# giuspugl/COSMOMAP2

Measured on AMD Instinct MI355X. Metric: TOD samples/s through P^T N^-1 P, higher is better.
Workload: dtype f64

## Files before the change

cosmomap2_amd/build.py:

```python
import glob
import os
import subprocess
import sys
from concurrent.futures import ThreadPoolExecutor

HERE = os.path.dirname(os.path.abspath(__file__))
CSRC = os.path.join(HERE, "csrc")
OBJ = os.path.join(HERE, "csrc", "build")
LIB = os.path.join(HERE, "libcosmomap2_hip.so")
ARCH = "gfx950"
HIPCC = os.environ.get("HIPCC", "/opt/rocm/bin/hipcc")
FLAGS = ["--offload-arch=" + ARCH, "-O3", "-fPIC", "-std=c++17", "-ffp-contract=off",
         "-fno-fast-math", "-Wall", "-Wno-unused-result", "-munsafe-fp-atomics"]


FMA_OK = {"cm2_overlap_save.hip"}


STAMP = os.path.join(HERE, "libcosmomap2_hip.sources.sha16")


def source_hash():
    import hashlib
    h = hashlib.sha256()
    files = sorted(glob.glob(os.path.join(CSRC, "*.hip")) + glob.glob(os.path.join(CSRC, "*.h")) +
                   glob.glob(os.path.join(HERE, "..", "include", "*.h")), key=os.path.basename)
    for f in files:
        h.update(os.path.basename(f).encode() + b"\0")
        h.update(open(f, "rb").read())
    return h.hexdigest()[:16]


def library_stamp():
    at_build = open(STAMP).read().strip() if os.path.exists(STAMP) else None
    if os.environ.get("CM2_LIB_PATH"):
        at_build = "variant:" + os.path.basename(os.environ["CM2_LIB_PATH"])
    return {"sources_sha16_at_build": at_build, "sources_sha16_now": source_hash(),
            "library_matches_sources": at_build is not None and at_build == source_hash()}


def _newer(target, deps):
    if not os.path.exists(target):
        return True
    t = os.path.getmtime(target)
    return any(os.path.getmtime(d) > t for d in deps)


def compile_command(src, obj):
    flags = list(FLAGS) + os.environ.get("CM2_EXTRA_HIPCC_FLAGS", "").split()
    if os.path.basename(src) in FMA_OK:
        flags[flags.index("-ffp-contract=off")] = "-ffp-contract=fast"
    return [HIPCC] + flags + ["-Rpass-analysis=kernel-resource-usage", "-c", src, "-o", obj]


def build(force=False, verbose=True, allow_spills=None):
    from cosmomap2_amd import kernel_resources as KR
    os.makedirs(OBJ, exist_ok=True)
    srcs = sorted(glob.glob(os.path.join(CSRC, "*.hip")))
    hdrs = glob.glob(os.path.join(CSRC, "*.h")) + \
        glob.glob(os.path.join(HERE, "..", "include", "*.h"))
    jobs = []
    objs = []
    for s in srcs:
        o = os.path.join(OBJ, os.path.basename(s)[:-4] + ".o")
        objs.append(o)
        res = os.path.join(OBJ, os.path.basename(s)[:-4] + ".resources.json")
        if force or _newer(o, [s] + hdrs) or not os.path.exists(res):
            jobs.append((s, compile_command(s, o)))
    for f in os.listdir(OBJ):
        stem = f.split(".")[0]
        if (f.endswith(".o") or f.endswith(".resources.json")) and \
                not os.path.exists(os.path.join(CSRC, stem + ".hip")):
            os.remove(os.path.join(OBJ, f))

    def run(job):
        src, cmd = job
        if verbose:
            print(" ".join(cmd), flush=True)
        p = subprocess.run(cmd, stderr=subprocess.PIPE, text=True)
        rest = [ln for ln in p.stderr.splitlines() if "-Rpass-analysis=kernel-resource-usage" not in ln]
        if rest and (verbose or p.returncode):
            print("\n".join(rest), file=sys.stderr, flush=True)
        if p.returncode:
            raise subprocess.CalledProcessError(p.returncode, cmd)
        KR.store(os.path.basename(src), p.stderr)

    if jobs:
        with ThreadPoolExecutor(max_workers=min(4, len(jobs))) as ex:
            list(ex.map(run, jobs))
    if jobs or force or _newer(LIB, objs):
        cmd = [HIPCC, "--offload-arch=" + ARCH, "-shared", "-o", LIB] + objs + \
            ["-L/opt/rocm/lib", "-lrocfft", "-Wl,-rpath,/opt/rocm/lib"]
        if verbose:
            print(" ".join(cmd), flush=True)
        subprocess.check_call(cmd)
        with open(STAMP, "w") as fh:
            fh.write(source_hash() + "\n")
    elif not os.path.exists(STAMP):
        with open(STAMP, "w") as fh:
            fh.write(source_hash() + "\n")
    rows = KR.load_all()
    if jobs:
        prof = os.path.join(HERE, "..", "profiles")
        if os.path.isdir(prof):
            with open(os.path.join(prof, "kernel_resources.md"), "w") as fh:
                fh.write("# Register / scratch / LDS use of every kernel in libcosmomap2_hip.so\n\n"
                         "Written by `cosmomap2_amd/build.py` from hipcc's `-Rpass-analysis=kernel-resource-usage` "
                         "remarks of the compile that produced the shipped objects (gfx950). The build fails "
                         "when a kernel matching `kernel_resources.NO_SPILL` spills.\n\n")
                fh.write(KR.table(KR.own_kernels(rows)) + "\n")
    bad = KR.offenders(rows)
    if bad:
        msg = "default-path kernels spill registers: " + ", ".join(
            "%s (%d VGPRs, %d SGPRs spilled, %d B/lane scratch)" % (
                r["kernel"], r.get("vgpr_spill", 0), r.get("sgpr_spill", 0),
                r.get("scratch_bytes_per_lane", 0)) for r in bad)
        if allow_spills if allow_spills is not None else os.environ.get("CM2_ALLOW_SPILLS"):
            print("WARNING: " + msg, file=sys.stderr)
        else:
            raise RuntimeError(msg)
    return LIB


if __name__ == "__main__":
    build(force="--force" in sys.argv)
    print(LIB)
```

cosmomap2_amd/csrc/cm2_overlap_save.hip:

```cpp
#include "cm2_overlap_save.h"

#include <hipcub/hipcub.hpp>
#include <cstring>
#include <memory>
#include <mutex>

using namespace cm2;

namespace {

constexpr double kCos32[32] = {1.0, 0.9807852804032304, 0.9238795325112867, 0.8314696123025452, 0.7071067811865476, 0.5555702330196022, 0.3826834323650898, 0.19509032201612828, 0.0, -0.19509032201612828, -0.3826834323650898, -0.5555702330196022, -0.7071067811865476, -0.8314696123025452, -0.9238795325112867, -0.9807852804032304, -1.0, -0.9807852804032304, -0.9238795325112867, -0.8314696123025452, -0.7071067811865476, -0.5555702330196022, -0.3826834323650898, -0.19509032201612828, 0.0, 0.19509032201612828, 0.3826834323650898, 0.5555702330196022, 0.7071067811865476, 0.8314696123025452, 0.9238795325112867, 0.9807852804032304};
constexpr double kSin32[32] = {0.0, 0.19509032201612828, 0.3826834323650898, 0.5555702330196022, 0.7071067811865476, 0.8314696123025452, 0.9238795325112867, 0.9807852804032304, 1.0, 0.9807852804032304, 0.9238795325112867, 0.8314696123025452, 0.7071067811865476, 0.5555702330196022, 0.3826834323650898, 0.19509032201612828, 0.0, -0.19509032201612828, -0.3826834323650898, -0.5555702330196022, -0.7071067811865476, -0.8314696123025452, -0.9238795325112867, -0.9807852804032304, -1.0, -0.9807852804032304, -0.9238795325112867, -0.8314696123025452, -0.7071067811865476, -0.5555702330196022, -0.3826834323650898, -0.19509032201612828};

__host__ __device__ constexpr int ilog2(int r) { return r <= 1 ? 0 : 1 + ilog2(r >> 1); }

template <int R>
__host__ __device__ constexpr int brev(int m)
{
    int out = 0;
    for (int b = 0; b < ilog2(R); ++b) out |= ((m >> b) & 1) << (ilog2(R) - 1 - b);
    return out;
}

template <class T> __device__ __forceinline__ T ld_list(const T *p) { return __builtin_nontemporal_load(p); }
// ... 302 lines not shown
            ca[i] = ab_own[o + i * kT];
            cb[i] = ab_prt[(PT - 1) * kT - o - i * kT];
        }
    };
    request(0);
    __builtin_amdgcn_sched_barrier(0);
#pragma unroll
    for (int j = 0; j < H; ++j) {
        wp[H + j] = zr[reg_slot<16>(H + j)];
        wp[j] = zi[reg_slot<16>(H + j)];
    }
    if (special) {
#pragma unroll
        for (int j = 0; j < H; ++j) {
            xbuf[t * H + j] = zr[reg_slot<16>(j)];
            xbuf[(8 + t) * H + j] = zi[reg_slot<16>(j)];
        }
    }
    __syncthreads();
    if (!special) {
        double *__restrict__ pp = buf + 33 * (263 - t) + 31;
#pragma unroll
        for (int m0 = 0; m0 < H; m0 += BP) {
            if (m0 > 0) request(m0);
#pragma unroll
            for (int i0 = 0; i0 < BP; i0 += 4) {
                double pre[4], pim[4];
#pragma unroll
                for (int i = 0; i < 4; ++i) {
                    pre[i] = pp[-(m0 + i0 + i)];
                    pim[i] = pp[-H - (m0 + i0 + i)];
                }
#pragma unroll
                for (int i = 0; i < 4; ++i) {
                    const int m = m0 + i0 + i, sl = reg_slot<16>(m);
                    const double a = ca[i0 + i].x, b = ca[i0 + i].y, ap = cb[i0 + i].x, bp = cb[i0 + i].y;
                    const double nr = a * zr[sl] + b * pim[i];
                    const double ni = a * zi[sl] + b * pre[i];
                    const double qr = ap * pre[i] + bp * zi[sl];
                    const double qi = ap * pim[i] + bp * zr[sl];
                    zr[sl] = nr;
                    zi[sl] = ni;
                    pp[-m] = qr;
                    pp[-H - m] = qi;
                }
            }
            __builtin_amdgcn_sched_barrier(0);
        }
    } else {
        const int tl = t == 0 ? 0 : 8 - t;
        const double *__restrict__ up = buf + 33 * (7 - t) + 47;
#pragma unroll
        for (int m0 = 0; m0 < H; m0 += BP) {
            if (m0 > 0) request(m0);
#pragma unroll
            for (int i = 0; i < BP; ++i) {
                const int m = m0 + i, sl = reg_slot<16>(m);
                const int ms = t == 0 ? (m == 0 ? 0 : H - m) : H - 1 - m;
                const double pre_ = xbuf[tl * H + ms], pim_ = xbuf[(8 + tl) * H + ms];
                const double nr = ca[i].x * zr[sl] + ca[i].y * pim_;
                const double ni = ca[i].x * zi[sl] + ca[i].y * pre_;
                zr[sl] = nr;
                zi[sl] = ni;
                const int mu = PT - 1 - m, su = reg_slot<16>(mu);
                const double ure = up[-mu], uim = up[-mu - H];
                zr[su] = cb[i].x * wp[mu] + cb[i].y * uim;
                zi[su] = cb[i].x * wp[mu - H] + cb[i].y * ure;
            }
            __builtin_amdgcn_sched_barrier(0);
        }
    }
    __syncthreads();
    if (!special) {
#pragma unroll
        for (int j = 0; j < H; ++j) {
            zr[reg_slot<16>(H + j)] = wp[H + j];
            zi[reg_slot<16>(H + j)] = wp[j];
        }
    }
    __syncthreads();
}


template <int PT, int MODE, bool BUF>
__global__ __launch_bounds__(kT, PT == 16 ? 4 : 2) void k_os_real(
    const WinDesc *__restrict__ wins, int nwin, const double2 *__restrict__ Wtw,
    const double2 *Wtw_inv, const double2 *__restrict__ AB, const uint32_t *__restrict__ lst_k,
    const uint16_t *__restrict__ lst_q, const ListHdr *__restrict__ hdrs,
    const uint32_t *__restrict__ tabs, int rmax, const double *__restrict__ v,
    double *__restrict__ out, uint32_t nbytes, const IListHdr *__restrict__ ihdrs,
    const uint32_t *__restrict__ iflags OS_STAMP_PARAM)
{
    using G = Geo<PT>;
    constexpr int N = G::N, H = PT / 2;
    __amdgpu_buffer_rsrc_t v_rs, o_rs;
    if constexpr (BUF) {
        v_rs = __builtin_amdgcn_make_buffer_rsrc(const_cast<double *>(v), 0, (int)nbytes, 0x00020000);
        o_rs = __builtin_amdgcn_make_buffer_rsrc(out, 0, (int)nbytes, 0x00020000);
    }
    auto gather = [&](uint32_t k) -> double {
        if constexpr (BUF) {
            const v2u_t r = __builtin_amdgcn_raw_buffer_load_b64(v_rs, k * 8u, 0, 0);
            return __builtin_bit_cast(double, r);
        } else {
            return ld_gather(v + (k != kInvalidSample ? k : 0u));
        }
    };
    auto keep = [&](uint32_t k, double x) -> double {
        if constexpr (BUF) return x;
        return k != kInvalidSample ? x : 0.0;
    };
    extern __shared__ double buf[];
    uint32_t *__restrict__ tab_lds = reinterpret_cast<uint32_t *>(buf + G::LDSD);
    const int t = threadIdx.x;
    const int per_xcd = (nwin + 7) / 8;
    const int win = (blockIdx.x & 7) * per_xcd + (blockIdx.x >> 3);
    if (win >= nwin) return;
    const WinDesc wd = wins[win];
    const int64_t w0 = wd.start - kHalo;
    const int wave = __builtin_amdgcn_readfirstlane(t >> 6);
    OS_STAMP(0);

    auto list_args = [&](int l) {
        ListArgs la;
        const int64_t e0 = (int64_t)win * G::PER + G::list_off(l);
        la.k = nullptr;
        la.q = nullptr;
        la.hdr = nullptr;
        la.tab = nullptr;
        if constexpr (MODE == 1) la.k = lst_k + e0;
        if constexpr (MODE == 1 || MODE == 2) la.q = lst_q + e0;
        if constexpr (MODE == 2) {
            la.hdr = hdrs + ((int64_t)win * G::NLIST + l);
            la.tab = tabs + ((int64_t)win * G::NLIST + l) * rmax;
        }
        return la;
    };

    double zr[PT], zi[PT];
    if constexpr (MODE == 0) {
#pragma unroll
        for (int h = 0; h < 2; ++h) {
            double vv[PT];
#pragma unroll
            for (int u = 0; u < PT; ++u) {
                const int64_t ts = w0 + (int64_t)h * N + t + u * kT;
                vv[u] = (ts >= wd.lo && ts < wd.hi) ? v[ts] : 0.0;
            }
#pragma unroll
            for (int u = 0; u < PT; ++u) buf[t + u * kT] = vv[u];
            __syncthreads();
            const double2 *__restrict__ sp = reinterpret_cast<const double2 *>(buf) + t;
#pragma unroll
            for (int m = 0; m < H; ++m) {
                const double2 p = sp[256 * m];
                zr[h * H + m] = p.x;
                zi[h * H + m] = p.y;
            }
            __syncthreads();
        }
    } else if constexpr (MODE == 3) {
        const IListHdr *__restrict__ h0 = ihdrs + (int64_t)win * 2;
        const uint32_t *__restrict__ pl = reinterpret_cast<const uint32_t *>(lst_q + (int64_t)win * G::PER);
        uint32_t fw[2], pp[PT];
        {
            tab_dma(tabs + ((int64_t)win * 2) * rmax, tab_lds, rmax, wave, t);
            fw[0] = iflags[((int64_t)win * 2) * 512 + t];
            fw[1] = iflags[((int64_t)win * 2) * 512 + 256 + t];
        }
        const uint32_t nv = h0->nvalid;
        const int wb0 = h0->wbase[wave], wb1 = h0->wbase[4 + wave];
#pragma unroll
        for (int m = 0; m < PT; ++m) pp[m] = pl[t + kT * m];
        __syncthreads();
        double va[PT], vb[PT];
        {
            uint32_t kk[PT];
            idecode<PT>(fw[0], tab_lds, wb0, nv, 0u, t, kk);
#pragma unroll
            for (int u = 0; u < PT; ++u) va[u] = keep(kk[u], gather(kk[u]));
        }
        __builtin_amdgcn_sched_barrier(0);
        {
            uint32_t kk[PT];
            idecode<PT>(fw[1], tab_lds, wb1, nv, (uint32_t)N, t, kk);
#pragma unroll
            for (int u = 0; u < PT; ++u) vb[u] = keep(kk[u], gather(kk[u]));
        }
        __builtin_amdgcn_sched_barrier(0);
#pragma unroll
        for (int j = 0; j < 2; ++j) {
#pragma unroll
            for (int u = 0; u < PT; ++u) buf[slot_of<PT>(t, u)] = j ? vb[u] : va[u];
            if (j == 1) {
                int tj = t;
                asm volatile("" : "+v"(tj));
#pragma unroll
                for (int m = 0; m < PT; ++m) pp[m] = pl[tj + kT * m];
            }
            __syncthreads();
#pragma unroll
            for (int m = 0; m < PT; ++m) {
                const uint32_t lo = (pp[m] & 0xFFFFu) - (uint32_t)(j * N), hi = (pp[m] >> 16) - (uint32_t)(j * N);
                const bool inl = lo < (uint32_t)N, inh = hi < (uint32_t)N;
                const double x = buf[inl ? lo : 0u], y = buf[inh ? hi : 0u];
                if (j == 0) {
                    zr[m] = inl ? x : 0.0;
                    zi[m] = inh ? y : 0.0;
                } else {
                    zr[m] = inl ? x : zr[m];
                    zi[m] = inh ? y : zi[m];
                }
            }
            __syncthreads();
        }
    } else {
        const ListArgs l0 = list_args(0), l1 = list_args(1);
        uint32_t qa[PT / 2], qb[PT / 2], ka[PT], kb[PT];
        uint32_t nva = 0, nvb = 0;
        int wba = -1, wbb = -1;
        if constexpr (MODE == 2) {
            nva = l0.hdr->nvalid;
            nvb = l1.hdr->nvalid;
            wba = l0.hdr->wbase[wave];
            wbb = l1.hdr->wbase[wave];
            tab_dma(l0.tab, tab_lds, rmax, wave, t);
            tab_dma(l1.tab, tab_lds + rmax, rmax, wave, t);
        }
        q_request<PT>(l0.q, t, qa);
        if constexpr (MODE == 1) {
#pragma unroll
            for (int u = 0; u < PT; ++u) ka[u] = ld_list(l0.k + slot_of<PT>(t, u));
        }
        q_request<PT>(l1.q, t, qb);
        if constexpr (MODE == 1) {
#pragma unroll
            for (int u = 0; u < PT; ++u) kb[u] = ld_list(l1.k + slot_of<PT>(t, u));
        }
        if constexpr (MODE == 2) {
            __syncthreads();
            OS_STAMP(6);
            rc_decode<PT>(qa, tab_lds, wba, nva, t, ka);
        }
        __builtin_amdgcn_sched_barrier(0);
        double va[PT], vv[PT];
        if constexpr (MODE == 2) rc_decode<PT>(qb, tab_lds + rmax, wbb, nvb, t, kb);
#pragma unroll
        for (int u = 0; u < PT; ++u) va[u] = gather(ka[u]);
#pragma unroll
        for (int u = 0; u < PT; ++u) vv[u] = gather(kb[u]);
        __builtin_amdgcn_sched_barrier(0);
#pragma unroll
        for (int u = 0; u < PT; ++u) buf[q_word(qa, u) & 0x7FFFu] = keep(ka[u], va[u]);
        OS_STAMP(7);
        __syncthreads();
        {
            const double2 *__restrict__ sp = reinterpret_cast<const double2 *>(buf) + t;
#pragma unroll
            for (int m = 0; m < H; ++m) {
                const double2 p = sp[256 * m];
                zr[m] = p.x;
                zi[m] = p.y;
            }
        }
        __syncthreads();
#pragma unroll
        for (int u = 0; u < PT; ++u) buf[q_word(qb, u) & 0x7FFFu] = keep(kb[u], vv[u]);
        __syncthreads();
        {
            const double2 *__restrict__ sp = reinterpret_cast<const double2 *>(buf) + t;
#pragma unroll
            for (int m = 0; m < H; ++m) {
                const double2 p = sp[256 * m];
                zr[H + m] = p.x;
                zi[H + m] = p.y;
            }
        }
        __syncthreads();
    }

    OS_STAMP(1);
    const double2 w_a = Wtw[t];
    const double2 w_b = Wtw[PT * (t & 15)];

    OS_XF(reg_fwd<PT, PT, 0>(zr, zi, w_a));
    OS_XF(reg_exchange<PT, 1, 2, PT>(zr, buf, t));
    OS_XF(reg_exchange<PT, 1, 2, PT>(zi, buf, t));
    OS_XF(reg_fwd<PT, 16, 0>(zr, zi, w_b));
    OS_XF(if constexpr (PT == 32) reg_fwd<PT, 16, 16>(zr, zi, w_b));
    OS_XF(reg_exchange<PT, 2, 3, 16>(zr, buf, t));
    OS_XF(reg_exchange<PT, 2, 3, 16>(zi, buf, t));
    const double2 *ab = AB + (int64_t)wd.blk * N + t;
    OS_XF(dft_sub<PT, 16, 0>(zr, zi));
    OS_XF(if constexpr (PT == 32) dft_sub<PT, 16, 16>(zr, zi));
    OS_STAMP(2);
    OS_XF(partner_filter_half<PT, (MODE == 1 && !BUF) ? 4 : 8>(zr, zi, buf, reinterpret_cast<double *>(tab_lds + 2 * rmax),
                                                               t, ab, AB + (int64_t)wd.blk * N));
    (void)ab;
    OS_STAMP(3);
    OS_XF(dit_sub<PT, 16, 0>(zi, zr));
    OS_XF(if constexpr (PT == 32) dit_sub<PT, 16, 16>(zi, zr));
    const double2 w_bi = Wtw_inv[PT * (t & 15)], w_ai = Wtw_inv[t];
    OS_XF(reg_exchange<PT, 3, 2, 0>(zr, buf, t));
    OS_XF(reg_exchange<PT, 3, 2, 0>(zi, buf, t));
    asm volatile("" : : "v"(w_bi.x), "v"(w_bi.y), "v"(w_ai.x), "v"(w_ai.y));
    __builtin_amdgcn_sched_barrier(0);
    if constexpr (MODE == 3) {
        constexpr int ER3 = G::RLEN / kT, NP = PT - 8;
        int l1 = 1;
        asm volatile("" : "+s"(l1));
        const IListHdr *h1 = ihdrs + (int64_t)win * 2 + l1;
        const uint32_t *tg = tabs + ((int64_t)win * 2 + l1) * rmax;
        const uint32_t *fg = iflags + ((int64_t)win * 2 + l1) * 512 + t;
        const uint32_t nv1 = h1->nvalid;
        uint32_t fr[G::RR], rp[NP];
        const uint32_t *rl = reinterpret_cast<const uint32_t *>(lst_q + (int64_t)win * G::PER + 2 * N);
        {
            tab_dma(tg, tab_lds + rmax, rmax, wave, t);
#pragma unroll
            for (int j = 0; j < G::RR; ++j) fr[j] = fg[256 * j];
            int t0 = t;
            asm volatile("" : "+v"(t0));
#pragma unroll
            for (int m = 0; m < NP; ++m) rp[m] = rl[t0 + kT * m];
        }
        __builtin_amdgcn_sched_barrier(0);
        OS_XF(reg_inv<PT, 16, 0>(zr, zi, w_bi));
        OS_XF(if constexpr (PT == 32) reg_inv<PT, 16, 16>(zr, zi, w_bi));
        OS_XF(reg_exchange<PT, 2, 1, 16>(zr, buf, t));
        OS_XF(reg_exchange<PT, 2, 1, 16>(zi, buf, t));
        OS_XF(reg_inv<PT, PT, 0>(zr, zi, w_ai));
        OS_STAMP(4);
#pragma unroll
        for (int j = 0; j < G::RR; ++j) {
            if (j > 0) {
                __syncthreads();
                int tj = t;
                asm volatile("" : "+v"(tj));
#pragma unroll
                for (int m = 0; m < NP; ++m) rp[m] = rl[tj + kT * m];
            }
#pragma unroll
            for (int m = 0; m < NP; ++m) {
                const uint32_t lo = (rp[m] & 0xFFFFu) - (uint32_t)(j * G::RLEN), hi = (rp[m] >> 16) - (uint32_t)(j * G::RLEN);
                buf[lo < (uint32_t)G::RLEN ? lo : (uint32_t)N] = zr[brev<PT>(m + 4)];
                buf[hi < (uint32_t)G::RLEN ? hi : (uint32_t)N + 1u] = zi[brev<PT>(m + 4)];
            }
            __syncthreads();
            uint32_t ks3[ER3];
            idecode<ER3>(fr[j], tab_lds + rmax, h1->wbase[4 * j + wave], nv1, (uint32_t)(j * G::RLEN), t, ks3);
            double rv[ER3];
#pragma unroll
            for (int u = 0; u < ER3; ++u) rv[u] = buf[slot_of<ER3>(t, u)];
#pragma unroll
            for (int u = 0; u < ER3; ++u) {
                if constexpr (BUF) {
                    __builtin_amdgcn_raw_buffer_store_b64(__builtin_bit_cast(v2u_t, rv[u]), o_rs, ks3[u] * 8u, 0, 0);
                } else {
                    if (ks3[u] != kInvalidSample) st_result(out + ks3[u], rv[u]);
                }
            }
        }
    } else {
    constexpr int ER = G::RLEN / kT;
    uint32_t qs[ER / 2], ks[ER];
    uint32_t nvs = 0;
    int wbs = -1;
    auto request_results = [&](int j, auto &qq, auto &kq, uint32_t &nv, int &wb, uint32_t *tdst) {
        if constexpr (MODE != 0) {
            int lj = 2 + j;
            asm volatile("" : "+s"(lj));
            const ListArgs ls = list_args(lj);
            if constexpr (MODE == 2) {
                nv = ls.hdr->nvalid;
                wb = ls.hdr->wbase[wave];
                tab_dma(ls.tab, tdst, rmax, wave, t);
            }
            q_request<ER>(ls.q, t, qq);
            (void)kq;
        }
    };
    constexpr bool EARLY = MODE == 2 || (MODE == 1 && BUF);
    uint32_t qs1[ER / 2];
    uint32_t nv1 = 0;
    int wb1 = -1;
    request_results(0, qs, ks, nvs, wbs, tab_lds);
    __builtin_amdgcn_sched_barrier(0);
    OS_XF(reg_inv<PT, 16, 0>(zr, zi, w_bi));
    OS_XF(if constexpr (PT == 32) reg_inv<PT, 16, 16>(zr, zi, w_bi));
    OS_XF(reg_exchange<PT, 2, 1, 16>(zr, buf, t));
    OS_XF(reg_exchange<PT, 2, 1, 16>(zi, buf, t));
    OS_XF(reg_inv<PT, PT, 0>(zr, zi, w_ai));
    OS_STAMP(4);
#pragma unroll
    for (int j = 0; j < G::RR; ++j) {
        const uint32_t *tabj = tab_lds + (EARLY && j > 0 ? rmax : 0);
        if (j > 0) {
            __syncthreads();
            if constexpr (EARLY) {
#pragma unroll
                for (int i = 0; i < ER / 2; ++i) qs[i] = qs1[i];
                nvs = nv1;
                wbs = wb1;
            } else {
                request_results(j, qs, ks, nvs, wbs, tab_lds);
                if constexpr (MODE == 2) __syncthreads();
            }
        }
        if constexpr (MODE == 2) rc_decode<ER>(qs, tabj, wbs, nvs, t, ks);
        double2 *__restrict__ sp = reinterpret_cast<double2 *>(buf) + t;
#pragma unroll
        for (int mm = 0; mm < G::RSLOTS; ++mm) {
            const int m = 4 + j * G::RSLOTS + mm;
            sp[256 * mm] = make_double2(zr[brev<PT>(m)], zi[brev<PT>(m)]);
        }
        if constexpr (MODE == 1) {
            const ListArgs ls = list_args(2 + j);
#pragma unroll
            for (int u = 0; u < ER; ++u) ks[u] = ld_list(ls.k + slot_of<ER>(t, u));
        }
        __syncthreads();
        if constexpr (EARLY)
            if (j + 1 < G::RR) request_results(j + 1, qs1, ks, nv1, wb1, tab_lds + rmax);
        if constexpr (MODE == 0) {
#pragma unroll
            for (int u = 0; u < ER; ++u) {
                const int e = t + u * kT;
                const int64_t o = (int64_t)j * G::RLEN + e;
                if (o < wd.len) out[wd.start + o] = buf[e];
            }
        } else {
            double rv[ER];
#pragma unroll
            for (int u = 0; u < ER; ++u) rv[u] = buf[q_word(qs, u) & 0x7FFFu];
#pragma unroll
            for (int u = 0; u < ER; ++u) {
                if constexpr (BUF) {
                    __builtin_amdgcn_raw_buffer_store_b64(__builtin_bit_cast(v2u_t, rv[u]), o_rs, ks[u] * 8u, 0, 0);
                } else {
                    if (ks[u] != kInvalidSample) st_result(out + ks[u], rv[u]);
                }
            }
        }
    }
    }
    OS_STAMP(5);
}

template <int PT>
__global__ __launch_bounds__(256) void k_real_keys(const WinDesc *__restrict__ wins, int64_t w0,
                                                    int64_t nw, const uint32_t *__restrict__ idx,
                                                    uint32_t *__restrict__ keys,
                                                    uint16_t *__restrict__ vals)
{
    using G = Geo<PT>;
    const int64_t total = nw * G::PER;
    const int64_t stride = (int64_t)gridDim.x * blockDim.x;
    for (int64_t g = (int64_t)blockIdx.x * blockDim.x + threadIdx.x; g < total; g += stride) {
        const int64_t p = g / G::PER;
        const int e = (int)(g - p * G::PER);
        const WinDesc wd = wins[w0 + p];
        uint32_t k = kInvalidSample;
        int val;
        if (e < 2 * G::N) {
            val = e & (G::N - 1);
            const int64_t ts = wd.start - kHalo + e;
            if (ts >= wd.lo && ts < wd.hi) k = idx[ts];
        } else {
            const int o = e - 2 * G::N;
            val = o % G::RLEN;
            if (o < wd.len) k = idx[wd.start + o];
        }
        keys[g] = k;
        vals[g] = (uint16_t)(val | (k == kInvalidSample ? 0x8000 : 0));
    }
}

template <int PT>
struct RealListOffset {
    int end;
    __host__ __device__ int operator()(int s) const
    {
        using G = Geo<PT>;
        const int l = s % G::NLIST + end;
        return (s / G::NLIST) * G::PER + (l == G::NLIST ? G::PER : G::list_off(l));
    }
};

template <int PT>
__global__ __launch_bounds__(256) void k_real_rc(int64_t nlists, const uint32_t *__restrict__ lk,
                                                  uint16_t *__restrict__ lq, ListHdr *__restrict__ hdrs,
                                                  uint32_t *__restrict__ tabs, int rmax,
                                                  uint32_t *__restrict__ max_runs)
{
    using G = Geo<PT>;
    __shared__ int wsum[4], vsum[4];
    const int64_t lid = blockIdx.x;
    if (lid >= nlists) return;
    const int l = (int)(lid % G::NLIST);
    const int64_t win = lid / G::NLIST;
    const int64_t e0 = win * G::PER + G::list_off(l);
    const int len = G::list_len(l);
    const int t = threadIdx.x, lane = t & 63, wave = t >> 6;
    int runs = 0, nvalid = 0;
    for (int s0 = 0; s0 < len; s0 += 256) {
        const int s = s0 + t;
        const uint32_t k = lk[e0 + s];
        const uint32_t prev = s > 0 ? lk[e0 + s - 1] : kInvalidSample;
        const bool valid = k != kInvalidSample;
        const bool flag = valid && (s == 0 || k != prev + 1u);
        const uint64_t fm = __ballot(flag), vm = __ballot(valid);
        const int below = __builtin_amdgcn_mbcnt_hi((uint32_t)(fm >> 32), __builtin_amdgcn_mbcnt_lo((uint32_t)fm, 0u));
        if (lane == 0) { wsum[wave] = __popcll(fm); vsum[wave] = __popcll(vm); }
        __syncthreads();
        int wbase = 0, tot = 0, vtot = 0;
#pragma unroll
        for (int w = 0; w < 4; ++w) {
            if (w < wave) wbase += wsum[w];
            tot += wsum[w];
            vtot += vsum[w];
        }
        __syncthreads();
        const int r = runs + wbase + below + (flag ? 1 : 0) - 1;
        if (flag) {
            if (r < rmax) tabs[lid * rmax + r] = k - (uint32_t)s;
        }
        const uint16_t q = lq[e0 + s];
        lq[e0 + s] = (uint16_t)((q & 0x7FFFu) | (flag ? 0x8000u : 0u));
        if (s % (len / 4) == 0) hdrs[lid].wbase[s / (len / 4)] = flag ? r - 1 : r;
// ... 288 lines not shown
__global__ void k_real_cos_table(int N, double *__restrict__ ct)
{
    const int m = blockIdx.x * blockDim.x + threadIdx.x;
    if (m <= N) ct[m] = cospi((double)m / (double)N);
}

constexpr int kSpecK = 1024;
__global__ __launch_bounds__(256) void k_real_spectrum(int nb, int64_t lambda, int N,
                                                        const double *__restrict__ bands,
                                                        const double *__restrict__ ct_g,
                                                        double *__restrict__ Hs)
{
    extern __shared__ double ct[];
    constexpr int PER = kSpecK / 256;
    const int chunks = (N + 1 + kSpecK - 1) / kSpecK;
    const int b = blockIdx.x / chunks, c = blockIdx.x % chunks;
    for (int m = threadIdx.x; m <= N; m += 256) ct[m] = ct_g[m];
    __syncthreads();
    const double *band = bands + (int64_t)b * lambda;
    const int mask = 2 * N - 1;
    int k[PER], m[PER];
    double acc[PER];
#pragma unroll
    for (int u = 0; u < PER; ++u) {
        k[u] = c * kSpecK + u * 256 + (int)threadIdx.x;
        m[u] = (int)(((lambda - 1) * (int64_t)k[u]) & mask);
        acc[u] = 0.0;
    }
    for (int64_t j = lambda - 1; j >= 1; --j) {
        const double a = band[j];
#pragma unroll
        for (int u = 0; u < PER; ++u) {
            const int f = m[u] <= N ? m[u] : 2 * N - m[u];
            acc[u] += a * ct[f];
            m[u] = (m[u] - k[u]) & mask;
        }
    }
#pragma unroll
    for (int u = 0; u < PER; ++u)
        if (k[u] <= N) Hs[(int64_t)b * (N + 1) + k[u]] = band[0] + 2.0 * acc[u];
}

template <int PT>
__global__ __launch_bounds__(256) void k_real_alpha_beta(int nb, const double *__restrict__ Hs,
                                                          double2 *__restrict__ AB)
{
    constexpr int N = Geo<PT>::N;
    const int64_t total = (int64_t)nb * N;
    const int64_t stride = (int64_t)gridDim.x * blockDim.x;
    for (int64_t e = (int64_t)blockIdx.x * blockDim.x + threadIdx.x; e < total; e += stride) {
        const int64_t b = e / N;
        const int a = (int)(e - b * N);
        const int d1 = a / 256, d2 = (a / 16) % 16, d3 = a % 16;
        const int k = d1 + PT * d2 + 16 * PT * d3;
        const double *h = Hs + b * (N + 1);
        const double hk = h[k], hp = h[N - k];
        const double S = 0.5 * (hk + hp), Dd = 0.5 * (hk - hp);
        const double th = (double)k / (double)N;
        const int t = a / PT, m = a % PT;
        AB[b * N + (int64_t)m * kT + t] = make_double2((S - Dd * sinpi(th)) / (double)N,
                                                        (Dd * cospi(th)) / (double)N);
    }
}


}

namespace cm2 {

constexpr int kPT = 32;
using G32 = Geo<kPT>;
constexpr size_t kListCache = 3;

struct OsLists {
    uint64_t plan_id = 0;
    int mode = 0;
    uint32_t *d_lst_k = nullptr;
    uint16_t *d_lst_q = nullptr;
    ListHdr *d_hdrs = nullptr;
    uint32_t *d_tabs = nullptr;
    IListHdr *d_ihdrs = nullptr;
    uint32_t *d_iflags = nullptr;
    int rmax = 0;
    double bytes_per_window = 0.0;
    ~OsLists()
    {
        void *ptrs[] = {d_lst_k, d_lst_q, d_hdrs, d_tabs, d_ihdrs, d_iflags};
        for (void *q : ptrs)
            if (q) (void)cm2::dev_free(q);
    }
};

struct FusedOS {
    int64_t nwin = 0;
    int64_t nb = 0;
    WinDesc *d_wins = nullptr;
    double2 *d_AB = nullptr;
    double2 *d_W = nullptr;
    int want_lists = 0;
    bool build_sort = false;
    bool flat = false;
    int64_t sort_chunk_windows = 0;
    std::mutex mu;
    std::vector<std::shared_ptr<OsLists>> cache;
};

void fused_os_destroy(FusedOS *f)
{
    if (!f) return;
    f->cache.clear();
    void *ptrs[] = {f->d_wins, f->d_AB, f->d_W};
    for (void *q : ptrs)
        if (q) (void)cm2::dev_free(q);
    delete f;
}

bool fused_os_supported(int64_t lambda) { return lambda >= 1 && lambda - 1 <= kHalo; }

int64_t fused_os_length(const FusedOS *f) { return f ? G32::N : 0; }

int fused_os_create(FusedOS **out, const double *d_bands, int64_t lambda, const std::vector<int64_t> &off,
                    hipStream_t stream)
{
    using G = G32;
    CM2_CHECK(out != nullptr, "fused_os_create: out is NULL");
    *out = nullptr;
    CM2_CHECK(fused_os_supported(lambda), "fused overlap-save supports lambda <= 2049, got %lld",
              (long long)lambda);
    FusedOS *f = new FusedOS();
    struct Guard { FusedOS *f; ~Guard() { if (f) fused_os_destroy(f); } } guard{f};
    if (const char *e = getenv("CM2_OS_LISTS")) {
        if (!strcmp(e, "plain")) f->want_lists = 1;
        else if (!strcmp(e, "rc")) f->want_lists = 2;
        else if (!strcmp(e, "inv")) f->want_lists = 3;
    }
    if (const char *e = getenv("CM2_OS_LIST_BUILD")) f->build_sort = strcmp(e, "sort") == 0;
    f->flat = getenv("CM2_OS_FLAT") != nullptr;
    if (const char *e = getenv("CM2_OS_LIST_CHUNK_PAIRS")) f->sort_chunk_windows = atoll(e);
    const int64_t nb = (int64_t)off.size() - 1;
    f->nb = nb;
    std::vector<WinDesc> wins;
    for (int64_t b = 0; b < nb; ++b)
        for (int64_t s0 = off[b]; s0 < off[b + 1]; s0 += G::HOP) {
            WinDesc wd;
            wd.start = s0;
            wd.len = off[b + 1] - s0 < G::HOP ? off[b + 1] - s0 : G::HOP;
            wd.lo = off[b];
            wd.hi = off[b + 1];
            wd.blk = (int32_t)b;
            wd.pad = 0;
            wins.push_back(wd);
        }
    f->nwin = (int64_t)wins.size();
    CM2_CHECK(f->nwin * 4 < ((int64_t)1 << 31), "fused overlap-save: too many windows (%lld)", (long long)f->nwin);
    CM2_HIP(cm2::dev_malloc(&f->d_wins, sizeof(WinDesc) * (wins.size() ? wins.size() : 1)));
    if (!wins.empty())
        CM2_HIP(cm2::upload(f->d_wins, wins.data(), sizeof(WinDesc) * wins.size(), nullptr));
    CM2_HIP(cm2::dev_malloc(&f->d_AB, sizeof(double2) * (nb > 0 ? nb : 1) * G::N));
    if (nb > 0) {
        DevTemp<double> Hs;
        CM2_HIP(Hs.alloc(nb * (G::N + 1)));
        DevTemp<double> ct;
        CM2_HIP(ct.alloc(G::N + 1));
        k_real_cos_table<<<(G::N + 256) / 256, 256, 0, stream>>>(G::N, ct);
        CM2_LAUNCH_OK();
        const size_t ct_lds = sizeof(double) * (G::N + 1);
        static size_t ct_granted[64] = {0};
        CM2_HIP(ensure_dynamic_lds((const void *)k_real_spectrum, ct_lds, ct_granted));
        const int chunks = (G::N + 1 + kSpecK - 1) / kSpecK;
        k_real_spectrum<<<(int)nb * chunks, 256, ct_lds, stream>>>((int)nb, lambda, G::N, d_bands, ct, Hs);
        CM2_LAUNCH_OK();
        k_real_alpha_beta<kPT><<<grid_for(nb * G::N), kBlock, 0, stream>>>((int)nb, Hs, f->d_AB);
        CM2_LAUNCH_OK();
        CM2_HIP(hipStreamSynchronize(stream));
    }
    CM2_HIP(cm2::dev_malloc(&f->d_W, sizeof(double2) * G::N));
    k_real_twiddles<<<(G::N + 255) / 256, 256, 0, stream>>>(G::N, f->d_W);
    CM2_LAUNCH_OK();
    CM2_HIP(hipStreamSynchronize(stream));
    guard.f = nullptr;
    *out = f;
    return 0;
}

template <int MODE, bool BUF>
static int os_launch_t(const FusedOS *f, const OsLists *ls, const double *d_v, double *d_out, uint32_t nbytes,
                       hipStream_t stream)
{
    using G = G32;
    const int rmax = ls ? ls->rmax : 0;
    const size_t lds = sizeof(double) * (size_t)G::LDSD + (MODE >= 2 ? sizeof(uint32_t) * 2 * (size_t)rmax : 0) + 2048;
    static size_t granted[64] = {0};
    CM2_HIP(ensure_dynamic_lds((const void *)k_os_real<kPT, MODE, BUF>, lds, granted));
    if (f->nwin == 0) return 0;
    const int grid = (int)(((f->nwin + 7) / 8) * 8);
    k_os_real<kPT, MODE, BUF><<<grid, kT, lds, stream>>>(
        f->d_wins, (int)f->nwin, f->d_W, f->d_W, f->d_AB, ls ? ls->d_lst_k : nullptr, ls ? ls->d_lst_q : nullptr,
        ls ? ls->d_hdrs : nullptr, ls ? ls->d_tabs : nullptr, rmax, d_v, d_out, nbytes, ls ? ls->d_ihdrs : nullptr,
        ls ? ls->d_iflags : nullptr OS_STAMP_ARG);
    CM2_LAUNCH_OK();
    return 0;
}

static int os_launch(const FusedOS *f, const OsLists *ls, int64_t nvalid, const double *d_v, double *d_out,
                     hipStream_t stream)
{
    if (f->nwin == 0) return 0;
    const bool buf = nvalid > 0 && nvalid * 8 < (int64_t)0xFFFFFFF0u && !f->flat;
    const uint32_t nbytes = buf ? (uint32_t)(nvalid * 8) : 0u;
    if (ls->mode == 1)
        return buf ? os_launch_t<1, true>(f, ls, d_v, d_out, nbytes, stream)
                   : os_launch_t<1, false>(f, ls, d_v, d_out, 0, stream);
    if (ls->mode == 3 && ls->rmax <= 8 * kT)
        return buf ? os_launch_t<3, true>(f, ls, d_v, d_out, nbytes, stream)
                   : os_launch_t<3, false>(f, ls, d_v, d_out, 0, stream);
    if (ls->mode == 2 && ls->rmax <= 8 * kT)
        return buf ? os_launch_t<2, true>(f, ls, d_v, d_out, nbytes, stream)
                   : os_launch_t<2, false>(f, ls, d_v, d_out, 0, stream);
    set_error("fused overlap-save: run table of %d words per list does not fit the kernel", ls->rmax);
    return 2;
}

int fused_os_apply(const FusedOS *f, const double *d_v, double *d_out, hipStream_t stream)
{
    return os_launch_t<0, false>(f, nullptr, d_v, d_out, 0, stream);
}

static int os_rmax(int64_t ntiles)
{
    using G = G32;
    int64_t bound = ntiles > 0 ? ntiles : G::N;
    if (bound > G::N) bound = G::N;
    const int rmax = (int)((bound + 63) / 64 * 64);
    return rmax < 64 ? 64 : rmax;
}

static int os_build_lists_direct(const FusedOS *f, OsLists *ls, const OsPlanView &pv, bool want_rc, hipStream_t stream)
{
    using G = G32;
    const int64_t total = f->nwin * G::PER;
    const int64_t nlists = f->nwin * G::NLIST;
    CM2_HIP(cm2::dev_malloc(&ls->d_lst_q, sizeof(uint16_t) * total));
    const int rmax = os_rmax(pv.ntiles);
    const bool rc = want_rc && rmax <= 8 * kT;
    const size_t lds = sizeof(uint32_t) * (size_t)(4 * pv.ntiles + 1 + 12) + sizeof(uint16_t) * (size_t)G::N;
    static size_t granted[64] = {0};
    DevTemp<uint32_t> d_max;
    CM2_HIP(d_max.alloc(1));
    CM2_HIP(hipMemsetAsync(d_max.p, 0, sizeof(uint32_t), stream));
    if (rc) {
        CM2_HIP(cm2::dev_malloc(&ls->d_hdrs, sizeof(ListHdr) * nlists));
        CM2_HIP(cm2::dev_malloc(&ls->d_tabs, sizeof(uint32_t) * nlists * rmax));
        CM2_HIP(ensure_dynamic_lds((const void *)k_real_lists<kPT, true>, lds, granted));
        k_real_lists<kPT, true><<<(unsigned)nlists, 256, lds, stream>>>(f->d_wins, nlists, pv.d_idx, pv.d_tile_off,
                                                                       (int)pv.ntiles, ls->d_lst_q, nullptr, ls->d_hdrs,
                                                                       ls->d_tabs, rmax, d_max);
    } else {
        CM2_HIP(cm2::dev_malloc(&ls->d_lst_k, sizeof(uint32_t) * total));
        CM2_HIP(ensure_dynamic_lds((const void *)k_real_lists<kPT, false>, lds, granted));
        k_real_lists<kPT, false><<<(unsigned)nlists, 256, lds, stream>>>(f->d_wins, nlists, pv.d_idx, pv.d_tile_off,
                                                                        (int)pv.ntiles, ls->d_lst_q, ls->d_lst_k, nullptr,
                                                                        nullptr, rmax, d_max);
    }
    CM2_LAUNCH_OK();
    uint32_t h_max = 0;
    CM2_HIP(cm2::download(&h_max, d_max.p, sizeof(uint32_t), stream));
    CM2_HIP(hipStreamSynchronize(stream));
    if (rc) {
        CM2_CHECK((int)h_max <= rmax, "fused overlap-save: a list has %u address runs, more than the %d pixel "
                  "tiles allow", h_max, rmax);
        ls->rmax = rmax;
        ls->mode = 2;
        ls->bytes_per_window = 2.0 * G::PER + G::NLIST * (sizeof(ListHdr) + 4.0 * h_max);
    } else {
        ls->mode = 1;
        ls->bytes_per_window = 6.0 * G::PER;
    }
    return 0;
// ... 46 lines not shown
        DevTemp<char> d_temp;
        CM2_HIP(keys_in.alloc(cw_max * G::PER));
        CM2_HIP(vals_in.alloc(cw_max * G::PER));
        hipcub::CountingInputIterator<int> seg_id(0);
        using OffsetIt = hipcub::TransformInputIterator<int, RealListOffset<kPT>, hipcub::CountingInputIterator<int>>;
        OffsetIt seg_begin(seg_id, RealListOffset<kPT>{0}), seg_end(seg_id, RealListOffset<kPT>{1});
        size_t tb = 0;
        CM2_HIP(hipcub::DeviceSegmentedRadixSort::SortPairs(
            nullptr, tb, keys_in.p, ls->d_lst_k, vals_in.p, ls->d_lst_q, (int)(cw_max * G::PER),
            (int)(G::NLIST * cw_max), seg_begin, seg_end, 0, 32, stream));
        CM2_HIP(d_temp.alloc(tb + 16));
        for (int64_t p0 = 0; p0 < f->nwin; p0 += chunk_w) {
            const int64_t nw = f->nwin - p0 < chunk_w ? f->nwin - p0 : chunk_w;
            k_real_keys<kPT><<<grid_for(nw * G::PER), kBlock, 0, stream>>>(f->d_wins, p0, nw, pv.d_idx, keys_in, vals_in);
            CM2_LAUNCH_OK();
            size_t tbc = tb;
            CM2_HIP(hipcub::DeviceSegmentedRadixSort::SortPairs(
                d_temp.p, tbc, keys_in.p, ls->d_lst_k + p0 * G::PER, vals_in.p, ls->d_lst_q + p0 * G::PER,
                (int)(nw * G::PER), (int)(G::NLIST * nw), seg_begin, seg_end, 0, 32, stream));
        }
        CM2_HIP(hipStreamSynchronize(stream));
    }
    ls->mode = 1;
    ls->bytes_per_window = 6.0 * G::PER;
    const int64_t nlists = f->nwin * G::NLIST;
    if (want_rc) {
        const int rmax = os_rmax(tile_runs);
        if (rmax <= 8 * kT) {
            DevTemp<uint32_t> d_max;
            CM2_HIP(d_max.alloc(1));
            CM2_HIP(hipMemsetAsync(d_max.p, 0, sizeof(uint32_t), stream));
            CM2_HIP(cm2::dev_malloc(&ls->d_hdrs, sizeof(ListHdr) * nlists));
            CM2_HIP(cm2::dev_malloc(&ls->d_tabs, sizeof(uint32_t) * nlists * rmax));
            k_real_rc<kPT><<<(unsigned)nlists, 256, 0, stream>>>(nlists, ls->d_lst_k, ls->d_lst_q, ls->d_hdrs,
                                                                ls->d_tabs, rmax, d_max);
            CM2_LAUNCH_OK();
            uint32_t h_max = 0;
            CM2_HIP(cm2::download(&h_max, d_max.p, sizeof(uint32_t), stream));
            CM2_HIP(hipStreamSynchronize(stream));
            CM2_CHECK((int)h_max <= rmax, "fused overlap-save: a list has %u address runs, more than the %d pixel "
                      "tiles allow", h_max, rmax);
            (void)cm2::dev_free(ls->d_lst_k);
            ls->d_lst_k = nullptr;
            ls->rmax = rmax;
            ls->mode = 2;
            ls->bytes_per_window = 2.0 * G::PER + G::NLIST * (sizeof(ListHdr) + 4.0 * h_max);
        }
    }
    k_real_qperm<kPT><<<(unsigned)nlists, 256, 0, stream>>>(nlists, ls->d_lst_q);
    CM2_LAUNCH_OK();
    CM2_HIP(hipStreamSynchronize(stream));
    return 0;
}

static int os_lists_for(FusedOS *f, const OsPlanView &pv, hipStream_t stream, std::shared_ptr<OsLists> *out)
{
    std::lock_guard<std::mutex> lock(f->mu);
    for (size_t i = 0; i < f->cache.size(); ++i)
        if (f->cache[i]->plan_id == pv.plan_id) {
            std::shared_ptr<OsLists> hit = f->cache[i];
            f->cache.erase(f->cache.begin() + (long)i);
            f->cache.insert(f->cache.begin(), hit);
            *out = hit;
            return 0;
        }
    const int want = f->want_lists ? f->want_lists : (pv.ntiles >= 768 ? 3 : 2);
    std::shared_ptr<OsLists> ls = std::make_shared<OsLists>();
    ls->plan_id = pv.plan_id;
    const bool direct = !f->build_sort && pv.d_tile_off && pv.ntiles > 0 && pv.ntiles <= 4096;
    CM2_CHECK(f->nwin * G32::NLIST < ((int64_t)1 << 31), "fused overlap-save: too many lists (%lld)",
              (long long)(f->nwin * G32::NLIST));
    if (f->nwin == 0) {
        ls->mode = 1;
    } else {
        int rc;
        if (!direct)
            rc = os_build_lists_sorted(f, ls.get(), pv, want >= 2, pv.ntiles, stream);
        else if (want == 3 && os_rmax(pv.ntiles) <= 8 * kT)
            rc = os_build_ilists(f, ls.get(), pv, stream);
        else
            rc = os_build_lists_direct(f, ls.get(), pv, want >= 2, stream);
        if (rc) return rc;
    }
    f->cache.insert(f->cache.begin(), ls);
    while (f->cache.size() > kListCache) f->cache.pop_back();
    *out = ls;
    return 0;
}

int fused_os_prepare_indexed(FusedOS *f, const OsPlanView &pv, hipStream_t stream)
{
    std::shared_ptr<OsLists> ls;
    return os_lists_for(f, pv, stream, &ls);
}

int fused_os_apply_indexed(FusedOS *f, const OsPlanView &pv, const double *d_v, double *d_out, hipStream_t stream)
{
    std::shared_ptr<OsLists> ls;
    if (int rc = os_lists_for(f, pv, stream, &ls)) return rc;
    return os_launch(f, ls.get(), pv.nvalid, d_v, d_out, stream);
}

double fused_os_tile_info(const FusedOS *f_, int *kernel)
{
    FusedOS *f = const_cast<FusedOS *>(f_);
    std::shared_ptr<OsLists> ls;
    if (f) {
        std::lock_guard<std::mutex> lock(f->mu);
        if (!f->cache.empty()) ls = f->cache.front();
    }
    if (kernel) {
        kernel[0] = f ? kPT : 0;
        kernel[1] = ls ? ls->mode : 0;
    }
    if (!f) return 0.0;
    const double hop = (double)G32::HOP, win = (double)G32::W;
    const double lists = ls && ls->bytes_per_window > 0 ? ls->bytes_per_window : 6.0 * (win + hop);
    return (lists + 8.0 * win + 8.0 * hop) / hop;
}

#ifdef CM2_OS_STAMPS
extern "C" int cm2_os_debug_stamps(unsigned long long *d_buf)
{
    g_os_stamps_host = d_buf;
    return 0;
}
#endif

}
```

Baseline: 69.75 billion.

## Make mode-2 overlap-save kernel persistent with next-window list prefetch

Turns the mode-2 overlap-save kernel into a persistent kernel. The grid is capped at the number of resident workgroups, found through an occupancy query, and each workgroup loops over a strided range of windows within its XCD slice. During the last result-scatter stage it issues the next window's table DMA, packed-list loads and header reads, so list fetch latency overlaps with compute. Kernel arguments are reloaded from the kernarg segment behind asm barriers to limit register pressure, and machine LICM is disabled for this unit so the compiler does not hoist those loads. The risks are extra register pressure, load imbalance across windows, and more complex control flow.

New measurement: 62.23 billion. 10.8% lower.

```diff
diff --git a/cosmomap2_amd/build.py b/cosmomap2_amd/build.py
--- a/cosmomap2_amd/build.py
+++ b/cosmomap2_amd/build.py
@@ -16,6 +16,8 @@
 
 FMA_OK = {"cm2_overlap_save.hip"}
 
+
+UNIT_FLAGS = {"cm2_overlap_save.hip": ["-mllvm", "-disable-machine-licm"]}
 
 STAMP = os.path.join(HERE, "libcosmomap2_hip.sources.sha16")
 
@@ -50,6 +52,7 @@
     flags = list(FLAGS) + os.environ.get("CM2_EXTRA_HIPCC_FLAGS", "").split()
     if os.path.basename(src) in FMA_OK:
         flags[flags.index("-ffp-contract=off")] = "-ffp-contract=fast"
+    flags += UNIT_FLAGS.get(os.path.basename(src), [])
     return [HIPCC] + flags + ["-Rpass-analysis=kernel-resource-usage", "-c", src, "-o", obj]
 
 
diff --git a/cosmomap2_amd/csrc/cm2_overlap_save.hip b/cosmomap2_amd/csrc/cm2_overlap_save.hip
--- a/cosmomap2_amd/csrc/cm2_overlap_save.hip
+++ b/cosmomap2_amd/csrc/cm2_overlap_save.hip
@@ -408,6 +408,25 @@
 }
 
 
+struct OsKernArgs {
+    const WinDesc *wins;
+    int nwin;
+    const double2 *Wtw, *Wtw_inv, *AB;
+    const uint32_t *lst_k;
+    const uint16_t *lst_q;
+    const ListHdr *hdrs;
+    const uint32_t *tabs;
+    int rmax;
+    const double *v;
+    double *out;
+    uint32_t nbytes;
+    const IListHdr *ihdrs;
+    const uint32_t *iflags;
+};
+
+#ifndef CM2_OS_PERSIST
+#define CM2_OS_PERSIST 1
+#endif
 template <int PT, int MODE, bool BUF>
 __global__ __launch_bounds__(kT, PT == 16 ? 4 : 2) void k_os_real(
     const WinDesc *__restrict__ wins, int nwin, const double2 *__restrict__ Wtw,
@@ -419,11 +438,19 @@
 {
     using G = Geo<PT>;
     constexpr int N = G::N, H = PT / 2;
+    constexpr bool PERSIST = MODE == 2 && CM2_OS_PERSIST;
     __amdgpu_buffer_rsrc_t v_rs, o_rs;
-    if constexpr (BUF) {
+    if constexpr (BUF && !PERSIST) {
         v_rs = __builtin_amdgcn_make_buffer_rsrc(const_cast<double *>(v), 0, (int)nbytes, 0x00020000);
         o_rs = __builtin_amdgcn_make_buffer_rsrc(out, 0, (int)nbytes, 0x00020000);
     }
+    auto kernargs = [&]() {
+        const __attribute__((address_space(4))) OsKernArgs *p =
+            (const __attribute__((address_space(4))) OsKernArgs *)__builtin_amdgcn_kernarg_segment_ptr();
+        asm volatile("" : "+s"(p));
+        return p;
+    };
+#define OS_T() do { if constexpr (PERSIST) asm volatile("" : "+v"(t)); } while (0)
     auto gather = [&](uint32_t k) -> double {
         if constexpr (BUF) {
             const v2u_t r = __builtin_amdgcn_raw_buffer_load_b64(v_rs, k * 8u, 0, 0);
@@ -438,18 +465,18 @@
     };
     extern __shared__ double buf[];
     uint32_t *__restrict__ tab_lds = reinterpret_cast<uint32_t *>(buf + G::LDSD);
-    const int t = threadIdx.x;
+    int t = threadIdx.x;
     const int per_xcd = (nwin + 7) / 8;
-    const int win = (blockIdx.x & 7) * per_xcd + (blockIdx.x >> 3);
-    if (win >= nwin) return;
-    const WinDesc wd = wins[win];
-    const int64_t w0 = wd.start - kHalo;
-    const int wave = __builtin_amdgcn_readfirstlane(t >> 6);
-    OS_STAMP(0);
-
-    auto list_args = [&](int l) {
+    int win = (blockIdx.x & 7) * per_xcd + (blockIdx.x >> 3);
+    const int step = PERSIST ? (int)(gridDim.x >> 3) : 0;
+    int wend = nwin;
+    if constexpr (PERSIST) wend = ((int)(blockIdx.x & 7) + 1) * per_xcd < nwin ? ((int)(blockIdx.x & 7) + 1) * per_xcd : nwin;
+    if (win >= wend) return;
+    int wave = __builtin_amdgcn_readfirstlane(t >> 6);
+
+    auto list_args = [&](int w, int l) {
         ListArgs la;
-        const int64_t e0 = (int64_t)win * G::PER + G::list_off(l);
+        const int64_t e0 = (int64_t)w * G::PER + G::list_off(l);
         la.k = nullptr;
         la.q = nullptr;
         la.hdr = nullptr;
@@ -457,11 +484,54 @@
         if constexpr (MODE == 1) la.k = lst_k + e0;
         if constexpr (MODE == 1 || MODE == 2) la.q = lst_q + e0;
         if constexpr (MODE == 2) {
-            la.hdr = hdrs + ((int64_t)win * G::NLIST + l);
-            la.tab = tabs + ((int64_t)win * G::NLIST + l) * rmax;
+            la.hdr = hdrs + ((int64_t)w * G::NLIST + l);
+            la.tab = tabs + ((int64_t)w * G::NLIST + l) * rmax;
         }
         return la;
     };
+
+    uint32_t qa[PT / 2], qb[PT / 2];
+    uint32_t nva = 0, nvb = 0;
+    int wba = -1, wbb = -1;
+    int32_t blk = 0;
+    uint32_t hw[5] = {0u, 0u, 0u, 0u, 0u};
+    auto request_window = [&](int w) {
+        {
+            const auto *ka = kernargs();
+            wins = ka->wins;
+            hdrs = ka->hdrs;
+            tabs = ka->tabs;
+            lst_q = ka->lst_q;
+            rmax = ka->rmax;
+        }
+        const ListArgs l0 = list_args(w, 0), l1 = list_args(w, 1);
+        tab_dma(l0.tab, tab_lds, rmax, wave, t);
+        tab_dma(l1.tab, tab_lds + rmax, rmax, wave, t);
+        q_request<PT>(l0.q, t, qa);
+        q_request<PT>(l1.q, t, qb);
+        int z = 0;
+        asm volatile("" : "+v"(z));
+        hw[0] = (&l0.hdr->nvalid)[z];
+        hw[1] = (&l1.hdr->nvalid)[z];
+        hw[2] = (uint32_t)(&l0.hdr->wbase[wave])[z];
+        hw[3] = (uint32_t)(&l1.hdr->wbase[wave])[z];
+        hw[4] = (uint32_t)(&wins[w].blk)[z];
+    };
+    if constexpr (PERSIST) request_window(win);
+    do {
+    if constexpr (PERSIST) {
+        asm volatile("" : "+v"(t));
+        wave = __builtin_amdgcn_readfirstlane(t >> 6);
+        const auto *ka = kernargs();
+        rmax = ka->rmax;
+        v = ka->v;
+        nbytes = ka->nbytes;
+        if constexpr (BUF) v_rs = __builtin_amdgcn_make_buffer_rsrc(const_cast<double *>(v), 0, (int)nbytes, 0x00020000);
+    }
+    const WinDesc wd = wins[win];
+    const int64_t w0 = wd.start - kHalo;
+    if constexpr (!PERSIST) blk = wd.blk;
+    OS_STAMP(0);
 
     double zr[PT], zi[PT];
     if constexpr (MODE == 0) {
@@ -541,10 +611,9 @@
             __syncthreads();
         }
     } else {
-        const ListArgs l0 = list_args(0), l1 = list_args(1);
-        uint32_t qa[PT / 2], qb[PT / 2], ka[PT], kb[PT];
-        uint32_t nva = 0, nvb = 0;
-        int wba = -1, wbb = -1;
+        const ListArgs l0 = list_args(win, 0), l1 = list_args(win, 1);
+        uint32_t ka[PT], kb[PT];
+        if constexpr (!PERSIST) {
         if constexpr (MODE == 2) {
             nva = l0.hdr->nvalid;
             nvb = l1.hdr->nvalid;
@@ -563,8 +632,16 @@
 #pragma unroll
             for (int u = 0; u < PT; ++u) kb[u] = ld_list(l1.k + slot_of<PT>(t, u));
         }
+        }
         if constexpr (MODE == 2) {
             __syncthreads();
+            if constexpr (PERSIST) {
+                nva = __builtin_amdgcn_readfirstlane(hw[0]);
+                nvb = __builtin_amdgcn_readfirstlane(hw[1]);
+                wba = (int)__builtin_amdgcn_readfirstlane(hw[2]);
+                wbb = (int)__builtin_amdgcn_readfirstlane(hw[3]);
+                blk = (int32_t)__builtin_amdgcn_readfirstlane(hw[4]);
+            }
             OS_STAMP(6);
             rc_decode<PT>(qa, tab_lds, wba, nva, t, ka);
         }
@@ -606,6 +683,13 @@
     }
 
     OS_STAMP(1);
+    OS_T();
+    if constexpr (PERSIST) {
+        const auto *ka = kernargs();
+        Wtw = ka->Wtw;
+        AB = ka->AB;
+        rmax = ka->rmax;
+    }
     const double2 w_a = Wtw[t];
     const double2 w_b = Wtw[PT * (t & 15)];
 
@@ -616,16 +700,30 @@
     OS_XF(if constexpr (PT == 32) reg_fwd<PT, 16, 16>(zr, zi, w_b));
     OS_XF(reg_exchange<PT, 2, 3, 16>(zr, buf, t));
     OS_XF(reg_exchange<PT, 2, 3, 16>(zi, buf, t));
-    const double2 *ab = AB + (int64_t)wd.blk * N + t;
+    const double2 *ab = AB + (int64_t)blk * N + t;
     OS_XF(dft_sub<PT, 16, 0>(zr, zi));
     OS_XF(if constexpr (PT == 32) dft_sub<PT, 16, 16>(zr, zi));
     OS_STAMP(2);
+    OS_T();
     OS_XF(partner_filter_half<PT, (MODE == 1 && !BUF) ? 4 : 8>(zr, zi, buf, reinterpret_cast<double *>(tab_lds + 2 * rmax),
-                                                               t, ab, AB + (int64_t)wd.blk * N));
+                                                               t, ab, AB + (int64_t)blk * N));
     (void)ab;
     OS_STAMP(3);
+    OS_T();
     OS_XF(dit_sub<PT, 16, 0>(zi, zr));
     OS_XF(if constexpr (PT == 32) dit_sub<PT, 16, 16>(zi, zr));
+    OS_T();
+    if constexpr (PERSIST) {
+        const auto *ka = kernargs();
+        Wtw_inv = ka->Wtw_inv;
+        lst_q = ka->lst_q;
+        hdrs = ka->hdrs;
+        tabs = ka->tabs;
+        rmax = ka->rmax;
+        out = ka->out;
+        nbytes = ka->nbytes;
+        if constexpr (BUF) o_rs = __builtin_amdgcn_make_buffer_rsrc(out, 0, (int)nbytes, 0x00020000);
+    }
     const double2 w_bi = Wtw_inv[PT * (t & 15)], w_ai = Wtw_inv[t];
     OS_XF(reg_exchange<PT, 3, 2, 0>(zr, buf, t));
     OS_XF(reg_exchange<PT, 3, 2, 0>(zi, buf, t));
@@ -696,7 +794,7 @@
         if constexpr (MODE != 0) {
             int lj = 2 + j;
             asm volatile("" : "+s"(lj));
-            const ListArgs ls = list_args(lj);
+            const ListArgs ls = list_args(win, lj);
             if constexpr (MODE == 2) {
                 nv = ls.hdr->nvalid;
                 wb = ls.hdr->wbase[wave];
@@ -718,6 +816,7 @@
     OS_XF(reg_exchange<PT, 2, 1, 16>(zi, buf, t));
     OS_XF(reg_inv<PT, PT, 0>(zr, zi, w_ai));
     OS_STAMP(4);
+    OS_T();
 #pragma unroll
     for (int j = 0; j < G::RR; ++j) {
         const uint32_t *tabj = tab_lds + (EARLY && j > 0 ? rmax : 0);
@@ -741,13 +840,25 @@
             sp[256 * mm] = make_double2(zr[brev<PT>(m)], zi[brev<PT>(m)]);
         }
         if constexpr (MODE == 1) {
-            const ListArgs ls = list_args(2 + j);
+            const ListArgs ls = list_args(win, 2 + j);
 #pragma unroll
             for (int u = 0; u < ER; ++u) ks[u] = ld_list(ls.k + slot_of<ER>(t, u));
         }
         __syncthreads();
         if constexpr (EARLY)
             if (j + 1 < G::RR) request_results(j + 1, qs1, ks, nv1, wb1, tab_lds + rmax);
+        if constexpr (PERSIST) {
+            if (j + 1 == G::RR) {
+                if (win + step < wend) {
+                    request_window(win + step);
+                } else {
+#pragma unroll
+                    for (int i = 0; i < PT / 2; ++i) qa[i] = qb[i] = 0u;
+#pragma unroll
+                    for (int i = 0; i < 5; ++i) hw[i] = 0u;
+                }
+            }
+        }
         if constexpr (MODE == 0) {
 #pragma unroll
             for (int u = 0; u < ER; ++u) {
@@ -771,6 +882,7 @@
     }
     }
     OS_STAMP(5);
+    } while (PERSIST && (win += step) < wend);
 }
 
 template <int PT>
@@ -1225,6 +1337,7 @@
     IListHdr *d_ihdrs = nullptr;
     uint32_t *d_iflags = nullptr;
     int rmax = 0;
+    int resident[2] = {0, 0};
     double bytes_per_window = 0.0;
     ~OsLists()
     {
@@ -1326,17 +1439,41 @@
     return 0;
 }
 
+static size_t os_lds_bytes(int mode, int rmax)
+{
+    return sizeof(double) * (size_t)G32::LDSD + (mode >= 2 ? sizeof(uint32_t) * 2 * (size_t)rmax : 0) + 2048;
+}
+
+template <bool BUF>
+static int os_resident_workgroups(int rmax, int *out)
+{
+    const size_t lds = os_lds_bytes(2, rmax);
+    static size_t granted[64] = {0};
+    CM2_HIP(ensure_dynamic_lds((const void *)k_os_real<kPT, 2, BUF>, lds, granted));
+    int dev = 0, cus = 0, per_cu = 0;
+    CM2_HIP(hipGetDevice(&dev));
+    CM2_HIP(hipDeviceGetAttribute(&cus, hipDeviceAttributeMultiprocessorCount, dev));
+    CM2_HIP(hipOccupancyMaxActiveBlocksPerMultiprocessor(&per_cu, (const void *)k_os_real<kPT, 2, BUF>, kT, lds));
+    CM2_CHECK(cus > 0 && per_cu > 0, "fused overlap-save: no resident workgroup (%d CUs x %d)", cus, per_cu);
+    *out = cus * per_cu;
+    return 0;
+}
+
 template <int MODE, bool BUF>
 static int os_launch_t(const FusedOS *f, const OsLists *ls, const double *d_v, double *d_out, uint32_t nbytes,
                        hipStream_t stream)
 {
-    using G = G32;
     const int rmax = ls ? ls->rmax : 0;
-    const size_t lds = sizeof(double) * (size_t)G::LDSD + (MODE >= 2 ? sizeof(uint32_t) * 2 * (size_t)rmax : 0) + 2048;
+    const size_t lds = os_lds_bytes(MODE, rmax);
     static size_t granted[64] = {0};
     CM2_HIP(ensure_dynamic_lds((const void *)k_os_real<kPT, MODE, BUF>, lds, granted));
     if (f->nwin == 0) return 0;
-    const int grid = (int)(((f->nwin + 7) / 8) * 8);
+    int grid = (int)(((f->nwin + 7) / 8) * 8);
+    if constexpr (MODE == 2 && CM2_OS_PERSIST) {
+        const int resident = ls->resident[BUF] / 8 * 8;
+        CM2_CHECK(resident >= 8, "fused overlap-save: %d resident workgroups", ls->resident[BUF]);
+        if (grid > resident) grid = resident;
+    }
     k_os_real<kPT, MODE, BUF><<<grid, kT, lds, stream>>>(
         f->d_wins, (int)f->nwin, f->d_W, f->d_W, f->d_AB, ls ? ls->d_lst_k : nullptr, ls ? ls->d_lst_q : nullptr,
         ls ? ls->d_hdrs : nullptr, ls ? ls->d_tabs : nullptr, rmax, d_v, d_out, nbytes, ls ? ls->d_ihdrs : nullptr,
@@ -1549,6 +1686,10 @@
             rc = os_build_lists_direct(f, ls.get(), pv, want >= 2, stream);
         if (rc) return rc;
     }
+    if (ls->mode == 2 && CM2_OS_PERSIST) {
+        if (int rc = os_resident_workgroups<false>(ls->rmax, &ls->resident[0])) return rc;
+        if (int rc = os_resident_workgroups<true>(ls->rmax, &ls->resident[1])) return rc;
+    }
     f->cache.insert(f->cache.begin(), ls);
     while (f->cache.size() > kListCache) f->cache.pop_back();
     *out = ls;
```
